# intellerce/controlanimate

Measured on AMD Instinct MI355X. Metric: frames_per_sec, higher is better.
Workload: dtype fp16

## Files before the change

### controlanimate_amd/_build.py

```python
from __future__ import annotations

import os
import subprocess
import sys
from concurrent.futures import ThreadPoolExecutor

CSRC = os.path.join(os.path.dirname(os.path.abspath(__file__)), "csrc")
LIB = os.path.join(CSRC, "libcontrolanimate_hip.so")
SOURCES = ["ca_gemm.hip", "ca_gemm_pp.hip", "ca_gemm_ar.hip", "ca_norm.hip", "ca_attention.hip", "ca_elementwise.hip", "ca_upscale.hip", "ca_color.hip", "ca_canny.hip", "ca_perceiver.hip", "ca_hed.hip", "ca_lineart.hip", "ca_mlsd.hip", "ca_softedge.hip", "ca_lineart_anime.hip", "ca_gfpgan.hip", "ca_depth.hip", "ca_openpose.hip", "ca_openpose_face.hip", "ca_openpose_hand.hip", "ca_normalbae.hip", "ca_retinaface.hip"]
HEADERS = ["ca_common.h", "ca_annot.h", "ca_gemm_core.h", "ca_gemm_plan.h", "ca_gemm_pp2.h", "ca_gemm_wres.h", "ca_gemm_ps.h", "ca_gemm_pq.h", "ca_gemm_ar.h", "ca_ff_fused.h", "ca_attn_out.h", "ca_tattn_fused.h", "ca_xattn_fused.h", "ca_gemm_seq.h", "ca_conv_wino.h", os.path.join("..", "..", "include", "controlanimate_hip.h")]
FLAGS = ["--offload-arch=gfx950", "-O3", "-std=c++17", "-fPIC", "-Wall", "-Wno-unused-function",
         "-mllvm", "-amdgpu-mfma-vgpr-form"]


EXTRA = {"ca_attention.hip": ["-fno-honor-nans"],
         "ca_color.hip": ["-ffp-contract=off"],
         "ca_hed.hip": ["-ffp-contract=off"],
         "ca_mlsd.hip": ["-ffp-contract=off"],
         "ca_softedge.hip": ["-ffp-contract=off"],
         "ca_gfpgan.hip": ["-ffp-contract=off"],
         "ca_depth.hip": ["-ffp-contract=off"],
         "ca_openpose.hip": ["-ffp-contract=off"]}
EXTRA["ca_openpose_face.hip"] = ["-ffp-contract=off"]
EXTRA["ca_openpose_hand.hip"] = ["-ffp-contract=off"]
EXTRA["ca_normalbae.hip"] = ["-ffp-contract=off"]
# ... 62 lines not shown
```

### controlanimate_amd/_capi.py

```python
from __future__ import annotations

import ctypes as C
import os

_HERE = os.path.dirname(os.path.abspath(__file__))
LIB_PATH = os.environ.get("CA_HIP_LIB") or os.path.join(_HERE, "csrc", "libcontrolanimate_hip.so")

CA_BF16, CA_F16 = 0, 1
CA_F32 = 2
CA_ACT_NONE, CA_ACT_SILU = 0, 1
CA_ACT_RELU = 4
CA_ACT_RELU6 = 5
CA_ACT_LEAKY02 = 6
CA_ACT_LEAKY001 = 7
CA_MLSD_TOPK = 200
CA_POSE_MAX_PEAKS, CA_POSE_MAX_PEOPLE, CA_POSE_AREA_TAPS = 64, 64, 8
CA_POSE_OVERFLOW_PEAKS, CA_POSE_OVERFLOW_PEOPLE = 1, 2
CA_POSE_OVERFLOW_FACES, CA_POSE_OVERFLOW_FACE_RESIZE = 4, 8
CA_FACE_SIZE, CA_FACE_HEAT, CA_FACE_PARTS, CA_FACE_MIN_SIDE, CA_FACE_SLOT_INTS = 384, 48, 71, 11, 8
CA_FACE_MODE_NONE, CA_FACE_MODE_LANCZOS4, CA_FACE_MODE_AREA = 0, 1, 2
CA_POSE_OVERFLOW_HANDS, CA_POSE_OVERFLOW_HAND_RESIZE = 16, 32
CA_HAND_PARTS, CA_HAND_HEAT_COLS, CA_HAND_MAP, CA_HAND_SCALES, CA_HAND_SLOT_INTS = 21, 24, 128, 4, 8
CA_HAND_MODE_NONE, CA_HAND_MODE_RESIZE, CA_HAND_MIN_BOX, CA_HAND_AREA_TAPS = 0, 1, 20, 16
CA_RFACE_MAX_CAND, CA_RFACE_HEAD_COLS, CA_RFACE_DET_COLS, CA_RFACE_MAX_FACES = 1024, 32, 15, 64
# ... 14 lines not shown
        ("a", C.c_void_p), ("a2", C.c_void_p), ("w", C.c_void_p), ("c", C.c_void_p),
        ("bias", C.c_void_p), ("rowbias", C.c_void_p), ("residual", C.c_void_p),
        ("lda", C.c_int64), ("lda2", C.c_int64), ("ldc", C.c_int64), ("ld_res", C.c_int64),
        ("ld_rowbias", C.c_int64),
        ("m", C.c_int32), ("n", C.c_int32), ("k1", C.c_int32), ("k2", C.c_int32),
        ("rows_per_group", C.c_int32),
        ("alpha", C.c_float), ("post_scale", C.c_float),
        ("act", C.c_int32), ("geglu", C.c_int32), ("out_f32", C.c_int32), ("dtype", C.c_int32),
        ("ln_stats", C.c_void_p), ("ln_colsum", C.c_void_p), ("ln_eps", C.c_float),
        ("workspace", C.c_void_p), ("workspace_bytes", C.c_int64),
        ("row_sums_out", C.c_void_p), ("ln_parts", C.c_int32),
        ("w_frag", C.c_void_p),
    ]


class FfArgs(C.Structure):
    _fields_ = [
        ("x", C.c_void_p), ("w1_frag", C.c_void_p), ("bias1", C.c_void_p), ("colsum1", C.c_void_p), ("ln_stats", C.c_void_p),
        ("w2_frag", C.c_void_p), ("bias2", C.c_void_p), ("residual", C.c_void_p), ("y", C.c_void_p),
        ("lda", C.c_int64), ("ldc", C.c_int64), ("ld_res", C.c_int64),
        ("m", C.c_int32), ("c", C.c_int32), ("inner", C.c_int32), ("ln_eps", C.c_float), ("dtype", C.c_int32),
        ("w_out_frag", C.c_void_p), ("bias_out", C.c_void_p), ("residual_out", C.c_void_p), ("ld_res_out", C.c_int64),
    ]


class TattnArgs(C.Structure):
    _fields_ = [
        ("x", C.c_void_p), ("w_frag", C.c_void_p), ("gamma", C.c_void_p), ("bias_pe", C.c_void_p), ("o", C.c_void_p),
        ("lda", C.c_int64), ("ldo", C.c_int64), ("ld_bias_pe", C.c_int64),
        ("batch", C.c_int32), ("frames", C.c_int32), ("tokens", C.c_int32), ("heads", C.c_int32), ("c", C.c_int32),
# ... 109 lines not shown


class Conv7x7Args(C.Structure):
    _fields_ = [
        ("x", C.c_void_p * 2), ("w", C.c_void_p * 2), ("bias", C.c_void_p * 2), ("y", C.c_void_p * 2),
        ("ldx", C.c_int64), ("ldy", C.c_int64),
        ("groups", C.c_int32), ("images", C.c_int32), ("h", C.c_int32), ("w_px", C.c_int32), ("cin", C.c_int32), ("cout", C.c_int32),
        ("relu", C.c_int32), ("dtype", C.c_int32),
    ]


SYMBOLS = {
    "ca_abi_version": (C.c_int, []),
    "ca_last_error": (C.c_char_p, []),
    "ca_gemm": (C.c_int, [C.POINTER(GemmArgs), C.c_void_p]),
    "ca_pack_w_frag": (C.c_int, [C.c_void_p, C.c_int32, C.c_int32, C.c_int32, C.c_void_p, C.c_void_p]),
    "ca_pack_w2_frag": (C.c_int, [C.c_void_p, C.c_int32, C.c_int32, C.c_void_p, C.c_void_p]),
    "ca_ff_fused": (C.c_int, [C.POINTER(FfArgs), C.c_void_p]),
    "ca_ff_fused_supported": (C.c_int, [C.POINTER(FfArgs)]),
    "ca_tattn_fused": (C.c_int, [C.POINTER(TattnArgs), C.c_void_p]),
    "ca_tattn_fused_supported": (C.c_int, [C.POINTER(TattnArgs)]),
    "ca_pack_w_tattn": (C.c_int, [C.c_void_p, C.c_int32, C.c_int32, C.c_void_p, C.c_void_p]),
    "ca_pack_w_out": (C.c_int, [C.c_void_p, C.c_int32, C.c_int32, C.c_void_p, C.c_void_p]),
    "ca_xattn_fused": (C.c_int, [C.POINTER(XattnArgs), C.c_void_p]),
    "ca_xattn_fused_supported": (C.c_int, [C.POINTER(XattnArgs)]),
    "ca_xattn_pack_w": (C.c_int, [C.c_void_p, C.c_int32, C.c_int32, C.c_void_p, C.c_void_p]),
    "ca_xattn_pack_kv": (C.c_int, [C.c_void_p, C.c_int64, C.c_int32, C.c_int32, C.c_int32, C.c_int32, C.c_float, C.c_int32, C.c_void_p, C.c_void_p]),
    "ca_gemm_ln_inline_supported": (C.c_int, [C.POINTER(GemmArgs)]),
    "ca_gemm_wants_finished_stats": (C.c_int, [C.POINTER(GemmArgs)]),
    "ca_ln_finish_sums": (C.c_int, [C.c_void_p, C.c_int, C.c_int64, C.c_int, C.c_float, C.c_void_p, C.c_void_p]),
# ... 174 lines not shown
```

### controlanimate_amd/context.py

```python
from __future__ import annotations

from dataclasses import dataclass, field
from typing import Optional

import torch


@dataclass
class ExecCtx:
    b: int
    f: int
    dtype: torch.dtype
    temb: torch.Tensor
    emb_groups: int
    ehs: Optional[torch.Tensor] = None
    frames_per_kv: int = 1
    kv_mod: int = 0
    gn_frames_per_stat: int = 1
    cache: dict = field(default_factory=dict)

    @property
    def images(self) -> int:
        return self.b * self.f

# ... 4 lines not shown
class Dispatch:
    gemm_ar = True
    ff_fused = True
    tattn_fused = True
    xattn_fused = True
    attn_out_fused = True
    xattn_ip_fused = True
    conv_winograd = True
    gn_winograd = True
    conv_up2_phase = True
    ln_row_sums = True
    repeat_kernel = True
    ln_fold = True
    cfg_shared = True
    cn_cfg_dedup = True
    pdc_block_fused = True
    dpt_head_fused = False
    pose_conv7_direct = True
    nbae_refine_fused = True
    controlnet_streams = 2


dispatch = Dispatch()
```

### controlanimate_amd/controlnet.py

```python
from __future__ import annotations

import dataclasses
from collections import OrderedDict

from typing import List, Optional, Sequence, Tuple, Union

import torch
from torch import nn

from . import kernels as K
from .context import ExecCtx
from .layers import HipConv1x1, HipConv3x3
from .unet import FrozenConfig, HipModelMixin, TimestepEmbedding, Timesteps
from .unet_blocks import UNetMidBlock3DCrossAttn, get_down_block


class ControlNetConditioningEmbedding(nn.Module):
    def __init__(self, conditioning_embedding_channels: int, conditioning_channels: int = 3,
                 block_out_channels: Tuple[int, ...] = (16, 32, 96, 256)):
        super().__init__()
        self.conv_in = HipConv3x3(conditioning_channels, block_out_channels[0])
        blocks = []
        for i in range(len(block_out_channels) - 1):
            blocks.append(HipConv3x3(block_out_channels[i], block_out_channels[i]))
# ... 173 lines not shown
            half = images // 2
            xh = self.conv_in.run(x[:half], residual=hint[:half])
            outs = [K.repeat_batch(xh)]
            x, o = first(xh, ctx, half_ctx=dataclasses.replace(ctx, b=half))
            outs += o
        else:
            x = self.conv_in.run(x, residual=hint)
            outs = [x]
        for blk in (self.down_blocks[1:] if shared else self.down_blocks):
            x, o = blk(x, ctx)
            outs += o
        x = self.mid_block(x, ctx)
        return outs, x, self.residual_scales(conditioning_scale, guess_mode), False

    @torch.no_grad()
    def apply_zero_convs(self, outs, x, scales, accumulate: Optional[Tuple[List[torch.Tensor], torch.Tensor]] = None, twice: bool = False):
        def one(zc, o, scale, prev):
            B_, h, w, c = o.shape
            rows = B_ * h * w
            a = o.view(rows, c)
            if not twice:
                return zc.run(a, alpha=scale, residual=None if prev is None else prev.view(rows, c)).view(B_, h, w, c)
            full = torch.empty((2 * B_, h, w, c), device=o.device, dtype=o.dtype)
            for hf in range(2):
                zc.run(a, alpha=scale, residual=None if prev is None else prev.view(2 * rows, c)[hf * rows:(hf + 1) * rows],
                       out=full.view(2 * rows, c)[hf * rows:(hf + 1) * rows])
            return full
        down = [one(zc, o, scales[i], None if accumulate is None else accumulate[0][i])
                for i, (zc, o) in enumerate(zip(self.controlnet_down_blocks, outs))]
        mid = one(self.controlnet_mid_block, x, scales[-1], None if accumulate is None else accumulate[1])
        return down, mid

    @torch.no_grad()
    def forward_nhwc(self, x: torch.Tensor, timestep, encoder_hidden_states: torch.Tensor, controlnet_cond: torch.Tensor,
                     conditioning_scale: float = 1.0, guess_mode: bool = False,
                     accumulate: Optional[Tuple[List[torch.Tensor], torch.Tensor]] = None, cfg_identical_halves: bool = False):
        outs, xm, scales, twice = self.forward_body(x, timestep, encoder_hidden_states, controlnet_cond, conditioning_scale, guess_mode,
                                                    cfg_identical_halves)
        return self.apply_zero_convs(outs, xm, scales, accumulate, twice)

    def forward(self, sample: torch.Tensor, timestep, encoder_hidden_states: torch.Tensor, controlnet_cond: torch.Tensor,
                conditioning_scale: float = 1.0, class_labels=None, timestep_cond=None, attention_mask=None,
                cross_attention_kwargs=None, guess_mode: bool = False, return_dict: bool = False):
        if not sample.is_cuda:
            raise RuntimeError("ControlNetModel runs on the HIP device only (no CPU fallback)")
# ... 22 lines not shown
        for n in self.nets:
            n.prepare(device, dtype)
        return self

    def forward_bodies(self, x, timestep, encoder_hidden_states, controlnet_cond: Sequence[torch.Tensor],
                       conditioning_scale: Sequence[float], guess_mode: bool = False, cfg_identical_halves: bool = False, streams=None):
        bodies = []
        for i, (net, cond, scale) in enumerate(zip(self.nets, controlnet_cond, conditioning_scale)):
            if streams:
                with torch.cuda.stream(streams[i % len(streams)]):
                    bodies.append(net.forward_body(x, timestep, encoder_hidden_states, cond, scale, guess_mode, cfg_identical_halves))
            else:
                bodies.append(net.forward_body(x, timestep, encoder_hidden_states, cond, scale, guess_mode, cfg_identical_halves))
        return bodies

    def finish(self, bodies, base: Optional[Tuple[List[torch.Tensor], torch.Tensor]] = None):
        acc = base
        for net, (outs, xm, scales, twice) in zip(self.nets, bodies):
            acc = net.apply_zero_convs(outs, xm, scales, acc, twice)
        return acc

    def forward_nhwc(self, x, timestep, encoder_hidden_states, controlnet_cond: Sequence[torch.Tensor],
                     conditioning_scale: Sequence[float], guess_mode: bool = False, cfg_identical_halves: bool = False):
        acc = None
        for net, cond, scale in zip(self.nets, controlnet_cond, conditioning_scale):
            acc = net.forward_nhwc(x, timestep, encoder_hidden_states, cond, scale, guess_mode, accumulate=acc,
                                   cfg_identical_halves=cfg_identical_halves)
        return acc

    def forward(self, sample, timestep, encoder_hidden_states, controlnet_cond, conditioning_scale, class_labels=None,
                timestep_cond=None, attention_mask=None, cross_attention_kwargs=None, guess_mode=False, return_dict=False):
        net0 = self.nets[0]
        net0._ensure_ready(sample.device)
        x = K.ncfhw_to_nhwc(sample.unsqueeze(2), net0.conv_in.cin_pad, net0.act_dtype)
# ... 3 lines not shown
```

### controlanimate_amd/controlresiduals_pipeline.py

```python
from __future__ import annotations

from typing import Callable, Dict, List, Optional, Sequence, Tuple

import numpy as np
import torch

from . import kernels as K
from .context import dispatch
from .controlnet import ControlNetModel, MultiControlNetModel


def _image_to_chw01(img) -> torch.Tensor:
    if torch.is_tensor(img):
        t = img.float()
        if t.dim() == 4:
            t = t[0]
        return t
    arr = np.asarray(img)
    if arr.ndim == 2:
        arr = np.stack([arr] * 3, axis=-1)
    t = torch.from_numpy(arr[..., :3].copy()).permute(2, 0, 1).float()
    return t / 255.0 if arr.dtype == np.uint8 else t


# ... 115 lines not shown
                                                    cfg_identical_halves=cfg_identical_halves, streams=streams if n_par > 1 else None)
            for s_ in streams[1:]:
                side.wait_stream(s_)
            if not capturing and n_par > 1:
                for i, (outs_, xm_, _, _) in enumerate(bodies):
                    if i % n_par:
                        for t_ in (*outs_, xm_):
                            t_.record_stream(side)
            if not fuse:
                down, mid = self.controlnet.finish(bodies)
                done = side.record_event()
        if not capturing:
            for s_ in streams:
                x_nhwc.record_stream(s_)

        def join(skips=None, mid_x=None):
            cur = torch.cuda.current_stream(dev)
            if not fuse:
                cur.wait_event(done)
                if not capturing:
                    for r in (*down, mid):
                        r.record_stream(cur)
                return down, mid
            if skips is None or mid_x is None:
                raise RuntimeError("a fused ControlNet join needs the UNet's skip tensors and mid-block output")
            side.wait_stream(cur)
            with torch.cuda.stream(side):
                d2, m2 = self.controlnet.finish(bodies, (list(skips), mid_x))
                fin = side.record_event()
            if not capturing:
                for s_ in (*skips, mid_x):
                    s_.record_stream(side)
            cur.wait_event(fin)
            if not capturing:
                for r in (*d2, m2):
                    r.record_stream(cur)
            return d2, m2

        join.fuse = fuse
        return join

    @torch.no_grad()
    def __call__(self, control_model_input: torch.Tensor, t, controlnet_prompt_embeds: torch.Tensor, frame_count: int,
                 image_embeds=None, do_classifier_free_guidance=True, guess_mode=True):
        b, c, f, h, w = control_model_input.shape
        if f != frame_count:
            raise ValueError("frame_count must equal the number of latent frames (SURVEY App. C-11)")
        net0 = self.controlnets[0]
        net0._ensure_ready(control_model_input.device)
        x = K.ncfhw_to_nhwc(control_model_input, net0.conv_in.cin_pad, net0.act_dtype)
        same = bool(self.detect_identical_halves and do_classifier_free_guidance and not guess_mode and b == 2
                    and torch.equal(control_model_input[0], control_model_input[1]))
        down, mid = self.residuals_nhwc(x, t, controlnet_prompt_embeds, guess_mode, cfg_identical_halves=same)

# ... 6 lines not shown
```

### controlanimate_amd/csrc/ca_gemm.hip

```cpp

#include "ca_gemm_plan.h"

namespace {
using namespace ca_gemm_detail;
#include "ca_conv_wino.h"

template <int DT, int BM, int BN, int WAVES_M, int WAVES_N, int MODE>
__global__ __launch_bounds__(256) void k_gemm(GemmKParams p) {
  constexpr int TM = BM / WAVES_M / 16;
  constexpr int TN = BN / WAVES_N / 16;
  constexpr int AI = BM / 32;
  constexpr int BI = BN / 32;
  static_assert(2 * (BM + BN) * BK >= BM * (BN + 8), "epilogue staging must fit");
  __shared__ __attribute__((aligned(16))) u16 smem[2 * (BM + BN) * BK];

  const int tid = threadIdx.x;
  const int lane = tid & 63;
  const int wid = tid >> 6;
  const int wm = wid / WAVES_N, wn = wid % WAVES_N;
  const int g = lane >> 4, l15 = lane & 15;

  const int tiles_n = (p.n + BN - 1) / BN;
  const unsigned bid = xcd_remap(blockIdx.x, gridDim.x);
  int tile_m, tile_n;
// ... 102 lines not shown
#pragma unroll
      for (int j = 0; j < TN; ++j) fb[j] = ld16(sb + lds_off(wn * TN * 16 + j * 16 + l15, s * 4 + g));
#pragma unroll
      for (int i = 0; i < TM; ++i)
#pragma unroll
        for (int j = 0; j < TN; ++j) acc[i][j] = Elem<DT>::mfma(fb[j], fa[i], acc[i][j]);
    }
    if (t + 1 < nt) store_tile(buf ^ 1);
    __syncthreads();
  }

  gemm_epilogue<DT, BM, BN, TM, TN>(p, acc, smem, m0, n0, wm, wn, l15, g, tid);
}


template <int DT, int BM, int BN, int WAVES_M, int WAVES_N, int MODE, int NBUF>
__global__ __launch_bounds__(256, NBUF == 1 ? (BN > 128 ? 3 : 4) : 2)
void k_gemm_dma(GemmKParams p) {
  static_assert(WAVES_M * WAVES_N == 4 && (NBUF == 1 || NBUF == 3), "instantiations: see above");
  constexpr int KT = BK;
  constexpr int CPR = KT / 8;
  constexpr int RPI = 64 / CPR;
  constexpr int NW = WAVES_M * WAVES_N, NT = NW * 64;
  constexpr int TM = BM / WAVES_M / 16;
  constexpr int TN = BN / WAVES_N / 16;
  constexpr int AG = BM / RPI / NW;
  constexpr int BG = BN / RPI / NW;
  constexpr int SMEM_ELEMS = NBUF * (BM + BN) * KT > BM * (BN + 8) ? NBUF * (BM + BN) * KT : BM * (BN + 8);
  auto swz = [](int row) { return (row >> 1) & 7; };
  auto lds_at = [&](int row, int chunk) { return row * KT + ((chunk ^ swz(row)) << 3); };
  __shared__ __attribute__((aligned(16))) u16 smem[SMEM_ELEMS];

  const int tid = threadIdx.x;
  const int lane = tid & 63;
  const int wid = tid >> 6;
  const int wm = wid / WAVES_N, wn = wid % WAVES_N;
  const int g = lane >> 4, l15 = lane & 15;

  const int tiles_n = (p.n + BN - 1) / BN;
  const int tiles_m = (p.m + BM - 1) / BM;
  unsigned bid = xcd_remap(blockIdx.x, gridDim.x);
  int split = 0;
  if (p.splits > 1) {
    split = bid / (unsigned)(tiles_m * tiles_n);
    bid -= split * (unsigned)(tiles_m * tiles_n);
  }
  int tile_m, tile_n;
  tile_coords(bid, tiles_m, tiles_n, tile_m, tile_n);
  const int m0 = tile_m * BM, n0 = tile_n * BN;

  const __amdgpu_buffer_rsrc_t rs_a = __builtin_amdgcn_make_buffer_rsrc((void*)p.a, 0, p.a_bytes, 0x00020000);
  const __amdgpu_buffer_rsrc_t rs_a2 = __builtin_amdgcn_make_buffer_rsrc((void*)(p.a2 ? p.a2 : p.a), 0, p.a2 ? p.a2_bytes : p.a_bytes, 0x00020000);
  const __amdgpu_buffer_rsrc_t rs_w = __builtin_amdgcn_make_buffer_rsrc((void*)p.w, 0, p.w_bytes, 0x00020000);

  const int r8 = lane / CPR, cp = lane % CPR;
  const int kc = p.c1 + p.c2;
// ... 130 lines not shown
  if (p.splits > 1) {
    float* slab = p.partial + (int64_t)split * p.m * p.n;
#pragma unroll
    for (int i = 0; i < TM; ++i) {
      const int m = m0 + wm * TM * 16 + i * 16 + l15;
      if (m >= p.m) continue;
#pragma unroll
      for (int j = 0; j < TN; ++j) {
        const int n = n0 + wn * TN * 16 + j * 16 + g * 4;
        if (n < p.n) *reinterpret_cast<f32x4*>(slab + (int64_t)m * p.n + n) = acc[i][j];
      }
    }
    return;
  }
  gemm_epilogue<DT, BM, BN, TM, TN, NT>(p, acc, smem, m0, n0, wm, wn, l15, g, tid);
}

template <int DT>
__global__ __launch_bounds__(256) void k_splitk_reduce(GemmKParams p) {
  const int64_t id = (int64_t)blockIdx.x * 256 + threadIdx.x;
  const int c8n = p.n >> 3;
  const int64_t m = id / c8n;
  if (m >= p.m) return;
  const int n = (int)(id - m * c8n) * 8;
  float v[8];
#pragma unroll
  for (int k = 0; k < 8; ++k) v[k] = 0.f;
  for (int sp = 0; sp < p.splits; ++sp) {
    const float* src = p.partial + ((int64_t)sp * p.m + m) * p.n + n;
    const f32x4 a = *reinterpret_cast<const f32x4*>(src), b = *reinterpret_cast<const f32x4*>(src + 4);
#pragma unroll
// ... 75 lines not shown
      return CA_OK;
  }
  CA_FAIL(CA_ERR_LAUNCH, "ca_gemm: no kernel for plan kind %d, tile %dx%d, %d stages", (int)g.kind, g.bm, g.bn, g.nbuf);
}

}

extern "C" int ca_gemm(const ca_gemm_args* a, void* stream) {
  DenseLaunch d;
  int rc = gemm_prepare(a, d);
  if (rc) return rc;
  hipStream_t st = (hipStream_t)stream;
  rc = a->dtype == CA_BF16 ? launch_gemm<CA_BF16, 0>(d.p, d.plan, st) : launch_gemm<CA_F16, 0>(d.p, d.plan, st);
  if (rc) return rc;
  CA_CHECK_LAUNCH("ca_gemm");
  return CA_OK;
}

extern "C" int64_t ca_gemm_workspace_bytes(const ca_gemm_args* a) {
  DenseLaunch d;
  return gemm_resolve(a, d) == CA_OK ? d.workspace : 0;
}

extern "C" int ca_gemm_row_sums_parts(const ca_gemm_args* a) {
  DenseLaunch d;
  DenseAsk ask{};
  ask.without_row_sums = true;
  return gemm_resolve(a, d, ask) == CA_OK ? row_sums_parts_of(d.p) : 0;
}

// ... 139 lines not shown
```

### controlanimate_amd/csrc/ca_gemm_core.h

```cpp
#pragma once
#include "ca_common.h"
#include <stdlib.h>

namespace ca_gemm_detail {


struct GemmKParams {
  const u16* a;
  const u16* a2;
  const u16* w;
  void* c;
  const float* bias;
  const float* rowbias;
  const float* ln_stats;
  const float* ln_colsum;
  const u16* res;
  int64_t lda, lda2, ldc, ld_res, ld_rowbias;
  unsigned a_bytes, a2_bytes, w_bytes;
  int m, n;
  int c1, c2;
  int taps;
  int kc_tiles;
  int hin, win, hout, wout, stride, ups, pad_lo;
  int rows_per_group;
// ... 2 lines not shown
  int splits;
  float* partial;
  int dbg;
  int tap_inner;
  float* row_sums;
  int ln_parts;
  int ln_inline;
  float ln_eps;
  const u16* wf;
  int w_group_rows;
  unsigned w_group_stride;
  int up2_rows, up2_tiles;
  unsigned up2_mag_w, up2_mag_h;
};

constexpr int BK = 64;

constexpr int GROUP_M = 8;
__device__ __forceinline__ void tile_coords(unsigned bid, int tiles_m, int tiles_n, int& tile_m, int& tile_n) {
  const unsigned gsz = GROUP_M * tiles_n;
  const unsigned group = bid / gsz, in = bid - group * gsz;
  const int first_m = group * GROUP_M;
  const int gm = tiles_m - first_m < GROUP_M ? tiles_m - first_m : GROUP_M;
  tile_m = first_m + in % gm;
  tile_n = in / gm;
}

__device__ __forceinline__ void k_tile_split(const GemmKParams& p, int t, int kct, int& tap, int& cc) {
  if (p.taps == 1) {
    tap = 0;
// ... 322 lines not shown
```

### controlanimate_amd/csrc/ca_gemm_plan.h

```cpp
#pragma once
#include "ca_gemm_core.h"

namespace ca_gemm_detail {

inline unsigned desc_bytes(int64_t elems) {
  const int64_t b = elems * 2;
  return (b > 0 && b < (int64_t)0xFFFFFF00ll) ? (unsigned)b : 0u;
}

inline bool dma_shape_ok(const GemmKParams& p) { return (p.c1 + p.c2) % BK == 0 && (p.c2 == 0 || p.c1 % BK == 0); }
inline bool dma_sizes_ok(const GemmKParams& p) { return p.a_bytes != 0 && p.w_bytes != 0 && (p.c2 == 0 || p.a2_bytes != 0); }
inline bool dma_capable(const GemmKParams& p) { return dma_shape_ok(p) && dma_sizes_ok(p); }

inline bool wres_eligible(const GemmKParams& p) {
  static const int wres_env = CA_KNOB("CA_GEMM_WRES", -1);
  const int kc = p.c1 + p.c2;
  return wres_env != 0 && kc == 320 && p.taps == 1 && (p.c2 == 0 || p.c1 % 32 == 0) && p.n % 160 == 0 && p.n / 160 <= 32 && !p.out_f32 &&
         p.splits <= 1 && !p.ln_parts && dma_sizes_ok(p) &&
         (!p.rowbias || p.rows_per_group % 32 == 0) &&
         act_out_fit31(p) &&
         (wres_env == 1 || p.m >= 16384);
}

inline bool ar_eligible(const GemmKParams& p, bool scratch) {
// ... 195 lines not shown
  if (p.ln_inline && p.wf) {
    if (ar_eligible(p, true)) d.workspace = (int64_t)p.m * 8;
    if (a->workspace && a->workspace_bytes >= (int64_t)p.m * 8) p.partial = reinterpret_cast<float*>(a->workspace);
  }
  d.plan = plan_gemm(p, 0);
  return CA_OK;
}

inline int gemm_prepare(const ca_gemm_args* a, DenseLaunch& d) {
  int rc = gemm_resolve(a, d);
  if (rc) return rc;
  CA_REQUIRE(!d.p.row_sums || row_sums_capable(d.p), "ca_gemm: row_sums_out is not available for this launch: ask ca_gemm_row_sums_parts() first");
  CA_REQUIRE(!d.p.ln_inline || wres_eligible(d.p), "ca_gemm: in-kernel LayerNorm statistics (ln_stats NULL) are not available for this launch: "
             "ask ca_gemm_ln_inline_supported() first and pass ln_stats otherwise");
  return CA_OK;
}

struct ConvGeom { int hl, wl, hout, wout; int64_t m; };
inline ConvGeom conv_geom(const ca_conv_args* a) {
  ConvGeom g;
  g.hl = a->hin << a->upsample, g.wl = a->win << a->upsample;
  const int pad = a->pad_asym ? 1 : 2;
  g.hout = (g.hl + pad - 3) / a->stride + 1;
  g.wout = (g.wl + pad - 3) / a->stride + 1;
  g.m = (int64_t)a->images * g.hout * g.wout;
  return g;
}
inline int64_t wino_tiles(const ca_conv_args* a, const ConvGeom& g) { return (int64_t)a->images * (g.hl / 2) * (g.wl / 2); }

inline int64_t wino_workspace_bytes(const ca_conv_args* a) {
// ... 118 lines not shown
```

### controlanimate_amd/kernels.py

```python
from __future__ import annotations

import ctypes as C
from typing import Optional

import torch

from . import _capi
from .context import dispatch
from ._capi import (AttnArgs, ConvArgs, ConvNarrowArgs, FfArgs, PerceiverAttnArgs, TattnArgs, XattnArgs, GemmArgs, GroupNormArgs, LayerNormArgs, CA_ACT_NONE,
                    CA_ACT_SILU, CA_BF16, CA_F16, check, lib)

ACT_NONE, ACT_SILU = CA_ACT_NONE, CA_ACT_SILU
ACT_QUICK_GELU, ACT_GELU = 2, 3
ACT_RELU = _capi.CA_ACT_RELU
ACT_RELU6 = _capi.CA_ACT_RELU6


def dt_code(dtype: torch.dtype) -> int:
    if dtype == torch.bfloat16:
        return CA_BF16
    if dtype == torch.float16:
        return CA_F16
    raise TypeError(f"activations must be bf16 or fp16, got {dtype}")

# ... 85 lines not shown
    if row_sums and dispatch.ln_row_sums and not geglu and not out_f32:
        parts = int(lib().ca_gemm_row_sums_parts(C.byref(args)))
        if parts > 0:
            rs = torch.empty((m, parts, 2), device=a.device, dtype=torch.float32)
            args.row_sums_out = _p(rs)
            out._row_sums = (rs, parts)
    wbytes = 0 if args.row_sums_out else int(lib().ca_gemm_workspace_bytes(C.byref(args)))
    if wbytes > 0:
        ws = torch.empty((wbytes,), device=a.device, dtype=torch.uint8)
        args.workspace, args.workspace_bytes = _p(ws), wbytes
    _record_plan(lib().ca_gemm_plan_name, args)
    check(lib().ca_gemm(C.byref(args), _stream()), "ca_gemm")
    return out


def attach_w_frag(w: torch.Tensor, geglu: bool = False) -> torch.Tensor:
    _req_cuda(w)
    if w.dim() != 2 or w.shape[1] != 320 or w.shape[0] % 320 != 0 or not w.is_contiguous() or w.dtype not in (torch.float16, torch.bfloat16):
        return w
    dst = torch.empty_like(w)
    check(lib().ca_pack_w_frag(w.data_ptr(), w.shape[0], w.shape[1], int(bool(geglu)), dst.data_ptr(), _stream()), "ca_pack_w_frag")
    w._frag = (dst, bool(geglu))
    return w


def ff_fused(x: torch.Tensor, w1_frag: torch.Tensor, bias1: torch.Tensor, colsum1: torch.Tensor, w2_frag: torch.Tensor,
             bias2: Optional[torch.Tensor], ln_eps: float, residual: Optional[torch.Tensor] = None,
             ln_stats: Optional[torch.Tensor] = None, *, w_out_frag: Optional[torch.Tensor] = None, bias_out: Optional[torch.Tensor] = None,
             residual_out: Optional[torch.Tensor] = None) -> Optional[torch.Tensor]:
    if not dispatch.ff_fused:
# ... 1845 lines not shown
```

### controlanimate_amd/unet.py

```python
from __future__ import annotations

from collections import OrderedDict

import dataclasses
import json
import os
from dataclasses import dataclass
from typing import Any, Dict, Optional, Tuple, Union

import torch
from torch import nn

from . import kernels as K
from .context import ExecCtx, dispatch
from .layers import HipGroupNorm, HipLinear, WeightArena, pack_concat_bias, pack_concat_rows
from .resnet import InflatedConv3d, InflatedGroupNorm, ResnetBlock3D
from .unet_blocks import UNetMidBlock3DCrossAttn, get_down_block, get_up_block


@dataclass
class UNet3DConditionOutput:
    sample: torch.Tensor


# ... 349 lines not shown
        shared = (cfg_identical_halves and dispatch.cfg_shared and b == 2 and getattr(first, "has_cross_attention", False) and
                  (not torch.is_tensor(timestep) or timestep.numel() == 1) and (timestep_cond is None or timestep_cond.shape[0] == 1))
        if shared:
            half_ctx = dataclasses.replace(ctx, b=1, temb=temb[:1], emb_groups=1)
            xh = self.conv_in.run(x[: x.shape[0] // 2])
            skips = [K.repeat_batch(xh)]
            x, outs = first(xh, ctx, half_ctx=half_ctx)
            skips += outs
        else:
            x = self.conv_in.run(x)
            skips = [x]
        for blk in (self.down_blocks[1:] if shared else self.down_blocks):
            x, outs = blk(x, ctx)
            skips += outs
        if callable(down_residuals) and getattr(down_residuals, "fuse", False):
            x = self.mid_block(x, ctx)
            skips, x = down_residuals(skips, x)
            for blk in self.up_blocks:
                n = len(blk.resnets)
                x = blk(x, skips[-n:], ctx)
                skips = skips[:-n]
            x = self.conv_norm_out.run(x, frames_per_stat=ctx.gn_frames_per_stat, act=K.ACT_SILU)
            return self.conv_out.run(x, out_f32=True)
        if callable(down_residuals):
            down_residuals, mid_residual = down_residuals()
        if down_residuals is not None:
            if len(down_residuals) != len(skips):
                raise ValueError("expected %d ControlNet residuals" % len(skips))
            skips = [K.add_bcast(s, r) for s, r in zip(skips, down_residuals)]
        x = self.mid_block(x, ctx)
# ... 72 lines not shown
```

### include/controlanimate_hip.h

```cpp
#ifndef CONTROLANIMATE_HIP_H
#define CONTROLANIMATE_HIP_H

#include <stdint.h>

#ifdef __cplusplus
extern "C" {
#endif

#define CA_ABI_VERSION 16

#define CA_BF16 0
#define CA_F16 1
#define CA_F32 2

#define CA_OK 0
#define CA_ERR_INVALID_ARG (-1)
#define CA_ERR_UNSUPPORTED (-2)
#define CA_ERR_LAUNCH (-3)

#define CA_ACT_NONE 0
#define CA_ACT_SILU 1
#define CA_ACT_QUICK_GELU 2
#define CA_ACT_GELU 3
#define CA_ACT_RELU 4
// ... 18 lines not shown
  float alpha, post_scale;
  int32_t act;
  int32_t geglu;
  int32_t out_f32;
  int32_t dtype;
  const float* ln_stats;
  const float* ln_colsum;
  float ln_eps;
  void* workspace;
  int64_t workspace_bytes;
  float* row_sums_out;
  int32_t ln_parts;
  const void* w_frag;
} ca_gemm_args;
int ca_gemm(const ca_gemm_args* args, void* stream);
int ca_pack_w_frag(const void* w, int32_t n, int32_t k, int32_t geglu, void* dst, void* stream);
typedef struct ca_ff_args {
  const void* x;
  const void* w1_frag;
  const float* bias1;
  const float* colsum1;
  const float* ln_stats;
  const void* w2_frag;
  const float* bias2;
  const void* residual;
  void* y;
  int64_t lda, ldc, ld_res;
  int32_t m, c, inner;
  float ln_eps;
  int32_t dtype;
// ... 542 lines not shown
```

Before: 15.91.

## Group ControlNet zero-conv GEMMs into one launch and start down-residuals early

```diff
diff --git a/controlanimate_amd/_build.py b/controlanimate_amd/_build.py
--- a/controlanimate_amd/_build.py
+++ b/controlanimate_amd/_build.py
@@ -8,7 +8,7 @@
 CSRC = os.path.join(os.path.dirname(os.path.abspath(__file__)), "csrc")
 LIB = os.path.join(CSRC, "libcontrolanimate_hip.so")
 SOURCES = ["ca_gemm.hip", "ca_gemm_pp.hip", "ca_gemm_ar.hip", "ca_norm.hip", "ca_attention.hip", "ca_elementwise.hip", "ca_upscale.hip", "ca_color.hip", "ca_canny.hip", "ca_perceiver.hip", "ca_hed.hip", "ca_lineart.hip", "ca_mlsd.hip", "ca_softedge.hip", "ca_lineart_anime.hip", "ca_gfpgan.hip", "ca_depth.hip", "ca_openpose.hip", "ca_openpose_face.hip", "ca_openpose_hand.hip", "ca_normalbae.hip", "ca_retinaface.hip"]
-HEADERS = ["ca_common.h", "ca_annot.h", "ca_gemm_core.h", "ca_gemm_plan.h", "ca_gemm_pp2.h", "ca_gemm_wres.h", "ca_gemm_ps.h", "ca_gemm_pq.h", "ca_gemm_ar.h", "ca_ff_fused.h", "ca_attn_out.h", "ca_tattn_fused.h", "ca_xattn_fused.h", "ca_gemm_seq.h", "ca_conv_wino.h", os.path.join("..", "..", "include", "controlanimate_hip.h")]
+HEADERS = ["ca_common.h", "ca_annot.h", "ca_gemm_core.h", "ca_gemm_plan.h", "ca_gemm_pp2.h", "ca_gemm_wres.h", "ca_gemm_ps.h", "ca_gemm_pq.h", "ca_gemm_ar.h", "ca_gemm_grouped.h", "ca_ff_fused.h", "ca_attn_out.h", "ca_tattn_fused.h", "ca_xattn_fused.h", "ca_gemm_seq.h", "ca_conv_wino.h", os.path.join("..", "..", "include", "controlanimate_hip.h")]
 FLAGS = ["--offload-arch=gfx950", "-O3", "-std=c++17", "-fPIC", "-Wall", "-Wno-unused-function",
          "-mllvm", "-amdgpu-mfma-vgpr-form"]
 
diff --git a/controlanimate_amd/_capi.py b/controlanimate_amd/_capi.py
--- a/controlanimate_amd/_capi.py
+++ b/controlanimate_amd/_capi.py
@@ -52,6 +52,15 @@
     ]
 
 
+class GemmGroupedProblem(C.Structure):
+    _fields_ = [
+        ("a", C.c_void_p), ("w", C.c_void_p), ("bias", C.c_void_p), ("c", C.c_void_p), ("residual", C.c_void_p),
+        ("c2", C.c_void_p), ("residual2", C.c_void_p),
+        ("lda", C.c_int64), ("ldc", C.c_int64), ("ld_res", C.c_int64), ("ldc2", C.c_int64), ("ld_res2", C.c_int64),
+        ("m", C.c_int32), ("n", C.c_int32), ("k", C.c_int32), ("alpha", C.c_float),
+    ]
+
+
 class FfArgs(C.Structure):
     _fields_ = [
         ("x", C.c_void_p), ("w1_frag", C.c_void_p), ("bias1", C.c_void_p), ("colsum1", C.c_void_p), ("ln_stats", C.c_void_p),
@@ -191,6 +200,9 @@
     "ca_abi_version": (C.c_int, []),
     "ca_last_error": (C.c_char_p, []),
     "ca_gemm": (C.c_int, [C.POINTER(GemmArgs), C.c_void_p]),
+    "ca_gemm_grouped": (C.c_int, [C.POINTER(GemmGroupedProblem), C.c_int32, C.c_int32, C.c_void_p]),
+    "ca_gemm_grouped_supported": (C.c_int, [C.POINTER(GemmGroupedProblem), C.c_int32, C.c_int32]),
+    "ca_gemm_grouped_plan_name": (C.c_int, [C.POINTER(GemmGroupedProblem), C.c_int32, C.c_int32, C.c_char_p, C.c_int32]),
     "ca_pack_w_frag": (C.c_int, [C.c_void_p, C.c_int32, C.c_int32, C.c_int32, C.c_void_p, C.c_void_p]),
     "ca_pack_w2_frag": (C.c_int, [C.c_void_p, C.c_int32, C.c_int32, C.c_void_p, C.c_void_p]),
     "ca_ff_fused": (C.c_int, [C.POINTER(FfArgs), C.c_void_p]),
diff --git a/controlanimate_amd/context.py b/controlanimate_amd/context.py
--- a/controlanimate_amd/context.py
+++ b/controlanimate_amd/context.py
@@ -42,6 +42,8 @@
     ln_fold = True
     cfg_shared = True
     cn_cfg_dedup = True
+    cn_zero_grouped = True
+    cn_zero_early = True
     pdc_block_fused = True
     dpt_head_fused = False
     pose_conv7_direct = True
diff --git a/controlanimate_amd/controlnet.py b/controlanimate_amd/controlnet.py
--- a/controlanimate_amd/controlnet.py
+++ b/controlanimate_amd/controlnet.py
@@ -211,21 +211,39 @@
         return outs, x, self.residual_scales(conditioning_scale, guess_mode), False
 
     @torch.no_grad()
-    def apply_zero_convs(self, outs, x, scales, accumulate: Optional[Tuple[List[torch.Tensor], torch.Tensor]] = None, twice: bool = False):
+    def apply_zero_convs(self, outs, x, scales, accumulate: Optional[Tuple[List[torch.Tensor], torch.Tensor]] = None, twice: bool = False,
+                         part: str = "all"):
+        from .context import dispatch
+        group = [] if dispatch.cn_zero_grouped else None
+
         def one(zc, o, scale, prev):
             B_, h, w, c = o.shape
             rows = B_ * h * w
             a = o.view(rows, c)
             if not twice:
-                return zc.run(a, alpha=scale, residual=None if prev is None else prev.view(rows, c)).view(B_, h, w, c)
+                res = None if prev is None else prev.view(rows, c)
+                if group is None:
+                    return zc.run(a, alpha=scale, residual=res).view(B_, h, w, c)
+                out = torch.empty((B_, h, w, c), device=o.device, dtype=o.dtype)
+                group.append(K.GroupedGemm(a, zc.w.t, zc.b.t, out.view(rows, c), res, alpha=scale))
+                return out
             full = torch.empty((2 * B_, h, w, c), device=o.device, dtype=o.dtype)
-            for hf in range(2):
-                zc.run(a, alpha=scale, residual=None if prev is None else prev.view(2 * rows, c)[hf * rows:(hf + 1) * rows],
-                       out=full.view(2 * rows, c)[hf * rows:(hf + 1) * rows])
+            halves = [(None if prev is None else prev.view(2 * rows, c)[hf * rows:(hf + 1) * rows], full.view(2 * rows, c)[hf * rows:(hf + 1) * rows])
+                      for hf in range(2)]
+            if group is None:
+                for res, out in halves:
+                    zc.run(a, alpha=scale, residual=res, out=out)
+            else:
+                group.append(K.GroupedGemm(a, zc.w.t, zc.b.t, halves[0][1], halves[0][0], halves[1][1], halves[1][0], alpha=scale))
             return full
-        down = [one(zc, o, scales[i], None if accumulate is None else accumulate[0][i])
-                for i, (zc, o) in enumerate(zip(self.controlnet_down_blocks, outs))]
-        mid = one(self.controlnet_mid_block, x, scales[-1], None if accumulate is None else accumulate[1])
+        down = mid = None
+        if part in ("all", "down"):
+            down = [one(zc, o, scales[i], None if accumulate is None else accumulate[0][i])
+                    for i, (zc, o) in enumerate(zip(self.controlnet_down_blocks, outs))]
+        if part in ("all", "mid"):
+            mid = one(self.controlnet_mid_block, x, scales[-1], None if accumulate is None else accumulate[1])
+        if group:
+            K.gemm_grouped(group)
         return down, mid
 
     @torch.no_grad()
@@ -278,10 +296,10 @@
                 bodies.append(net.forward_body(x, timestep, encoder_hidden_states, cond, scale, guess_mode, cfg_identical_halves))
         return bodies
 
-    def finish(self, bodies, base: Optional[Tuple[List[torch.Tensor], torch.Tensor]] = None):
+    def finish(self, bodies, base: Optional[Tuple[List[torch.Tensor], torch.Tensor]] = None, part: str = "all"):
         acc = base
         for net, (outs, xm, scales, twice) in zip(self.nets, bodies):
-            acc = net.apply_zero_convs(outs, xm, scales, acc, twice)
+            acc = net.apply_zero_convs(outs, xm, scales, acc, twice, part)
         return acc
 
     def forward_nhwc(self, x, timestep, encoder_hidden_states, controlnet_cond: Sequence[torch.Tensor],
diff --git a/controlanimate_amd/controlresiduals_pipeline.py b/controlanimate_amd/controlresiduals_pipeline.py
--- a/controlanimate_amd/controlresiduals_pipeline.py
+++ b/controlanimate_amd/controlresiduals_pipeline.py
@@ -153,6 +153,17 @@
             for s_ in streams:
                 x_nhwc.record_stream(s_)
 
+        early = {}
+
+        def start_down(skips):
+            cur = torch.cuda.current_stream(dev)
+            side.wait_stream(cur)
+            with torch.cuda.stream(side):
+                early["down"], _ = self.controlnet.finish(bodies, (list(skips), None), part="down")
+            if not capturing:
+                for s_ in skips:
+                    s_.record_stream(side)
+
         def join(skips=None, mid_x=None):
             cur = torch.cuda.current_stream(dev)
             if not fuse:
@@ -165,7 +176,11 @@
                 raise RuntimeError("a fused ControlNet join needs the UNet's skip tensors and mid-block output")
             side.wait_stream(cur)
             with torch.cuda.stream(side):
-                d2, m2 = self.controlnet.finish(bodies, (list(skips), mid_x))
+                if "down" in early:
+                    d2 = early.pop("down")
+                    _, m2 = self.controlnet.finish(bodies, (None, mid_x), part="mid")
+                else:
+                    d2, m2 = self.controlnet.finish(bodies, (list(skips), mid_x))
                 fin = side.record_event()
             if not capturing:
                 for s_ in (*skips, mid_x):
@@ -177,6 +192,7 @@
             return d2, m2
 
         join.fuse = fuse
+        join.start_down = start_down if fuse and dispatch.cn_zero_early else None
         return join
 
     @torch.no_grad()
diff --git a/controlanimate_amd/csrc/ca_gemm.hip b/controlanimate_amd/csrc/ca_gemm.hip
--- a/controlanimate_amd/csrc/ca_gemm.hip
+++ b/controlanimate_amd/csrc/ca_gemm.hip
@@ -140,9 +140,9 @@
 }
 
 
-template <int DT, int BM, int BN, int WAVES_M, int WAVES_N, int MODE, int NBUF>
-__global__ __launch_bounds__(256, NBUF == 1 ? (BN > 128 ? 3 : 4) : 2)
-void k_gemm_dma(GemmKParams p) {
+template <int DT, int BM, int BN, int WAVES_M, int WAVES_N, int MODE, int NBUF, bool SECOND = false>
+__device__ __forceinline__ void gemm_dma_tile(const GemmKParams& p, unsigned bid_raw, unsigned nblocks, void* c2 = nullptr, const u16* res2 = nullptr,
+                                              int64_t ldc2 = 0, int64_t ld_res2 = 0) {
   static_assert(WAVES_M * WAVES_N == 4 && (NBUF == 1 || NBUF == 3), "instantiations: see above");
   constexpr int KT = BK;
   constexpr int CPR = KT / 8;
@@ -165,7 +165,7 @@
 
   const int tiles_n = (p.n + BN - 1) / BN;
   const int tiles_m = (p.m + BM - 1) / BM;
-  unsigned bid = xcd_remap(blockIdx.x, gridDim.x);
+  unsigned bid = xcd_remap(bid_raw, nblocks);
   int split = 0;
   if (p.splits > 1) {
     split = bid / (unsigned)(tiles_m * tiles_n);
@@ -326,7 +326,21 @@
     return;
   }
   gemm_epilogue<DT, BM, BN, TM, TN, NT>(p, acc, smem, m0, n0, wm, wn, l15, g, tid);
-}
+  if (SECOND && c2) {
+    GemmKParams q = p;
+    q.c = c2, q.res = res2, q.ldc = ldc2, q.ld_res = ld_res2;
+    __syncthreads();
+    gemm_epilogue<DT, BM, BN, TM, TN, NT>(q, acc, smem, m0, n0, wm, wn, l15, g, tid);
+  }
+}
+
+template <int DT, int BM, int BN, int WAVES_M, int WAVES_N, int MODE, int NBUF>
+__global__ __launch_bounds__(256, NBUF == 1 ? (BN > 128 ? 3 : 4) : 2)
+void k_gemm_dma(GemmKParams p) {
+  gemm_dma_tile<DT, BM, BN, WAVES_M, WAVES_N, MODE, NBUF>(p, blockIdx.x, gridDim.x);
+}
+
+#include "ca_gemm_grouped.h"
 
 template <int DT>
 __global__ __launch_bounds__(256) void k_splitk_reduce(GemmKParams p) {
@@ -432,6 +446,30 @@
   rc = a->dtype == CA_BF16 ? launch_gemm<CA_BF16, 0>(d.p, d.plan, st) : launch_gemm<CA_F16, 0>(d.p, d.plan, st);
   if (rc) return rc;
   CA_CHECK_LAUNCH("ca_gemm");
+  return CA_OK;
+}
+
+extern "C" int ca_gemm_grouped_supported(const ca_gemm_grouped_problem* probs, int32_t count, int32_t dtype) {
+  GroupedTable t;
+  return grouped_capable(probs, count, dtype, t) ? 1 : 0;
+}
+
+extern "C" int ca_gemm_grouped(const ca_gemm_grouped_problem* probs, int32_t count, int32_t dtype, void* stream) {
+  GroupedTable t;
+  CA_REQUIRE(grouped_capable(probs, count, dtype, t), "ca_gemm_grouped: %d problems of dtype %d the grouped launch does not take (1..%d problems, fp16 / bf16, N and K "
+             "multiples of 64, leading dimensions multiples of 8, 16-byte aligned operands below 2 GB): ask ca_gemm_grouped_supported() first and run ca_gemm per "
+             "problem otherwise", count, dtype, GROUPED_MAX);
+  int rc = launch_gemm_grouped(t, dtype, (hipStream_t)stream);
+  if (rc) return rc;
+  CA_CHECK_LAUNCH("ca_gemm_grouped");
+  return CA_OK;
+}
+
+extern "C" int ca_gemm_grouped_plan_name(const ca_gemm_grouped_problem* probs, int32_t count, int32_t dtype, char* buf, int32_t len) {
+  CA_REQUIRE(buf && len > 0, "ca_gemm_grouped_plan_name: buffer");
+  GroupedTable t;
+  CA_REQUIRE(grouped_capable(probs, count, dtype, t), "ca_gemm_grouped_plan_name: problems the grouped launch does not take");
+  snprintf(buf, (size_t)len, "grouped128x64_r3");
   return CA_OK;
 }
 
diff --git a/controlanimate_amd/csrc/ca_gemm_core.h b/controlanimate_amd/csrc/ca_gemm_core.h
--- a/controlanimate_amd/csrc/ca_gemm_core.h
+++ b/controlanimate_amd/csrc/ca_gemm_core.h
@@ -40,6 +40,39 @@
   unsigned up2_mag_w, up2_mag_h;
 };
 
+constexpr int GROUPED_MAX = 32;
+struct GroupedProblem {
+  const u16* a;
+  const u16* w;
+  const float* bias;
+  u16* c;
+  const u16* res;
+  u16* c2;
+  const u16* res2;
+  int m, n, k;
+  int lda, ldc, ld_res, ldc2, ld_res2;
+  float alpha;
+};
+struct GroupedTable {
+  GroupedProblem prob[GROUPED_MAX];
+  unsigned first[GROUPED_MAX + 1];
+  int count;
+};
+static_assert(sizeof(GroupedTable) <= 3584, "the grouped table is a kernel argument: well under 4 KB");
+__host__ __device__ inline void grouped_fill(const GroupedProblem& g, GemmKParams& p) {
+  p = GemmKParams{};
+  p.a = g.a, p.w = g.w, p.c = g.c, p.bias = g.bias, p.res = g.res;
+  p.lda = g.lda, p.ldc = g.ldc, p.ld_res = g.ld_res;
+  p.a_bytes = (unsigned)(((int64_t)(g.m - 1) * g.lda + g.k) * 2);
+  p.w_bytes = (unsigned)((int64_t)g.n * g.k * 2);
+  p.m = g.m, p.n = g.n, p.c1 = g.k;
+  p.taps = 1;
+  p.kc_tiles = g.k / 64;
+  p.rows_per_group = 1;
+  p.alpha = g.alpha, p.post = 1.f;
+  p.splits = 1;
+}
+
 constexpr int BK = 64;
 
 constexpr int GROUP_M = 8;
diff --git a/controlanimate_amd/csrc/ca_gemm_grouped.h b/controlanimate_amd/csrc/ca_gemm_grouped.h
--- /dev/null
+++ b/controlanimate_amd/csrc/ca_gemm_grouped.h
@@ -0,0 +1,21 @@
+
+template <int DT>
+__global__ __launch_bounds__(256, 2) void k_gemm_grouped(GroupedTable t) {
+  const unsigned b = blockIdx.x;
+  int g = 0;
+#pragma unroll
+  for (int step = GROUPED_MAX / 2; step > 0; step >>= 1)
+    if (t.first[g + step] <= b) g += step;
+  g = __builtin_amdgcn_readfirstlane(g);
+  const GroupedProblem& q = t.prob[g];
+  GemmKParams p;
+  grouped_fill(q, p);
+  gemm_dma_tile<DT, 128, 64, 4, 1, 0, 3, true>(p, b - t.first[g], t.first[g + 1] - t.first[g], q.c2, q.res2, q.ldc2, q.ld_res2);
+}
+
+static int launch_gemm_grouped(const GroupedTable& t, int dtype, hipStream_t st) {
+  const dim3 grid(t.first[t.count]);
+  if (dtype == CA_BF16) hipLaunchKernelGGL((k_gemm_grouped<CA_BF16>), grid, dim3(256), 0, st, t);
+  else hipLaunchKernelGGL((k_gemm_grouped<CA_F16>), grid, dim3(256), 0, st, t);
+  return CA_OK;
+}
diff --git a/controlanimate_amd/csrc/ca_gemm_plan.h b/controlanimate_amd/csrc/ca_gemm_plan.h
--- a/controlanimate_amd/csrc/ca_gemm_plan.h
+++ b/controlanimate_amd/csrc/ca_gemm_plan.h
@@ -233,6 +233,52 @@
   CA_REQUIRE(!d.p.ln_inline || wres_eligible(d.p), "ca_gemm: in-kernel LayerNorm statistics (ln_stats NULL) are not available for this launch: "
              "ask ca_gemm_ln_inline_supported() first and pass ln_stats otherwise");
   return CA_OK;
+}
+
+inline bool grouped_problem_ok(const ca_gemm_grouped_problem& a, GroupedProblem& g) {
+  if (!a.a || !a.w || !a.c || a.m <= 0 || a.n <= 0 || a.k <= 0 || a.n % 64 != 0 || a.k % BK != 0) return false;
+  if (a.residual2 && !a.c2) return false;
+  const int64_t lds[5] = {a.lda, a.ldc, a.residual ? a.ld_res : 8, a.c2 ? a.ldc2 : 8, a.residual2 ? a.ld_res2 : 8};
+  for (int64_t ld : lds)
+    if (ld <= 0 || ld % 8 != 0 || ld >= (1ll << 31)) return false;
+  if (a.lda < a.k || a.ldc < a.n || (a.residual && a.ld_res < a.n) || (a.c2 && a.ldc2 < a.n) || (a.residual2 && a.ld_res2 < a.n)) return false;
+  if ((((uintptr_t)a.a | (uintptr_t)a.w | (uintptr_t)a.c | (uintptr_t)a.residual | (uintptr_t)a.c2 | (uintptr_t)a.residual2) & 15) != 0) return false;
+  if (((uintptr_t)a.bias & 15) != 0) return false;
+  g.a = (const u16*)a.a, g.w = (const u16*)a.w, g.bias = a.bias, g.c = (u16*)a.c, g.res = (const u16*)a.residual;
+  g.c2 = (u16*)a.c2, g.res2 = (const u16*)a.residual2;
+  g.m = a.m, g.n = a.n, g.k = a.k;
+  g.lda = (int)a.lda, g.ldc = (int)a.ldc, g.ld_res = a.residual ? (int)a.ld_res : 0;
+  g.ldc2 = a.c2 ? (int)a.ldc2 : 0, g.ld_res2 = a.residual2 ? (int)a.ld_res2 : 0;
+  g.alpha = a.alpha;
+  if (((int64_t)(a.m - 1) * a.lda + a.k) * 2 >= FIT31 || (int64_t)a.n * a.k * 2 >= FIT31) return false;
+  GemmKParams p;
+  grouped_fill(g, p);
+  if (!dma_capable(p) || !act_out_fit31(p) || p.w_bytes >= FIT31) return false;
+  if (g.c2) {
+    p.c = g.c2, p.res = g.res2, p.ldc = g.ldc2, p.ld_res = g.ld_res2;
+    if (!act_out_fit31(p)) return false;
+  }
+  return true;
+}
+inline bool grouped_capable(const ca_gemm_grouped_problem* probs, int count, int dtype, GroupedTable& t) {
+  if (!probs || count < 1 || count > GROUPED_MAX || (dtype != CA_F16 && dtype != CA_BF16)) return false;
+  int order[GROUPED_MAX];
+  for (int i = 0; i < count; ++i) {
+    int j = i;
+    for (; j > 0 && probs[order[j - 1]].m < probs[i].m; --j) order[j] = order[j - 1];
+    order[j] = i;
+  }
+  t = GroupedTable{};
+  t.count = count;
+  int64_t total = 0;
+  for (int i = 0; i < count; ++i) {
+    if (!grouped_problem_ok(probs[order[i]], t.prob[i])) return false;
+    t.first[i] = (unsigned)total;
+    total += (int64_t)ceil_div_i(t.prob[i].m, 128) * (t.prob[i].n / 64);
+    if (total >= (1ll << 31)) return false;
+  }
+  for (int i = count; i <= GROUPED_MAX; ++i) t.first[i] = (unsigned)total;
+  return true;
 }
 
 struct ConvGeom { int hl, wl, hout, wout; int64_t m; };
diff --git a/controlanimate_amd/kernels.py b/controlanimate_amd/kernels.py
--- a/controlanimate_amd/kernels.py
+++ b/controlanimate_amd/kernels.py
@@ -123,6 +123,47 @@
     return out
 
 
+class GroupedGemm:
+    __slots__ = ("a", "w", "bias", "out", "residual", "out2", "residual2", "alpha")
+
+    def __init__(self, a, w, bias, out, residual=None, out2=None, residual2=None, alpha: float = 1.0):
+        self.a, self.w, self.bias, self.out, self.residual, self.out2, self.residual2, self.alpha = a, w, bias, out, residual, out2, residual2, float(alpha)
+
+
+def gemm_grouped(problems) -> bool:
+    problems = list(problems)
+    if not problems:
+        return True
+    dt = problems[0].a.dtype
+    arr = (_capi.GemmGroupedProblem * len(problems))()
+    for g, q in zip(arr, problems):
+        _req_cuda(q.a, q.w, q.bias, q.out, q.residual, q.out2, q.residual2)
+        assert q.a.dim() == 2 and q.a.stride(1) == 1 and q.w.dim() == 2 and q.w.is_contiguous() and q.a.dtype == dt and q.w.dtype == dt
+        m, k = q.a.shape
+        n = q.w.shape[0]
+        assert q.w.shape[1] == k and (q.bias is None or (q.bias.dtype == torch.float32 and q.bias.numel() == n))
+        assert q.out2 is not None or q.residual2 is None
+        for t in (q.out, q.residual, q.out2, q.residual2):
+            assert t is None or (tuple(t.shape) == (m, n) and t.stride(1) == 1 and t.dtype == dt)
+        g.a, g.w, g.bias, g.c, g.residual, g.c2, g.residual2 = _p(q.a), _p(q.w), _p(q.bias), _p(q.out), _p(q.residual), _p(q.out2), _p(q.residual2)
+        g.lda, g.ldc = q.a.stride(0), q.out.stride(0)
+        g.ld_res = q.residual.stride(0) if q.residual is not None else 0
+        g.ldc2 = q.out2.stride(0) if q.out2 is not None else 0
+        g.ld_res2 = q.residual2.stride(0) if q.residual2 is not None else 0
+        g.m, g.n, g.k, g.alpha = m, n, k, q.alpha
+    if lib().ca_gemm_grouped_supported(arr, len(problems), dt_code(dt)):
+        if _plan_sink is not None:
+            buf = C.create_string_buffer(64)
+            _plan_sink.append(buf.value.decode() if lib().ca_gemm_grouped_plan_name(arr, len(problems), dt_code(dt), buf, 64) == 0 else "?")
+        check(lib().ca_gemm_grouped(arr, len(problems), dt_code(dt), _stream()), "ca_gemm_grouped")
+        return True
+    for q in problems:
+        gemm(q.a, q.w, bias=q.bias, residual=q.residual, alpha=q.alpha, out=q.out)
+        if q.out2 is not None:
+            gemm(q.a, q.w, bias=q.bias, residual=q.residual2, alpha=q.alpha, out=q.out2)
+    return False
+
+
 def attach_w_frag(w: torch.Tensor, geglu: bool = False) -> torch.Tensor:
     _req_cuda(w)
     if w.dim() != 2 or w.shape[1] != 320 or w.shape[0] % 320 != 0 or not w.is_contiguous() or w.dtype not in (torch.float16, torch.bfloat16):
diff --git a/controlanimate_amd/unet.py b/controlanimate_amd/unet.py
--- a/controlanimate_amd/unet.py
+++ b/controlanimate_amd/unet.py
@@ -387,6 +387,8 @@
             x, outs = blk(x, ctx)
             skips += outs
         if callable(down_residuals) and getattr(down_residuals, "fuse", False):
+            if getattr(down_residuals, "start_down", None) is not None:
+                down_residuals.start_down(skips)
             x = self.mid_block(x, ctx)
             skips, x = down_residuals(skips, x)
             for blk in self.up_blocks:
diff --git a/include/controlanimate_hip.h b/include/controlanimate_hip.h
--- a/include/controlanimate_hip.h
+++ b/include/controlanimate_hip.h
@@ -56,6 +56,21 @@
   const void* w_frag;
 } ca_gemm_args;
 int ca_gemm(const ca_gemm_args* args, void* stream);
+typedef struct ca_gemm_grouped_problem {
+  const void* a;
+  const void* w;
+  const float* bias;
+  void* c;
+  const void* residual;
+  void* c2;
+  const void* residual2;
+  int64_t lda, ldc, ld_res, ldc2, ld_res2;
+  int32_t m, n, k;
+  float alpha;
+} ca_gemm_grouped_problem;
+int ca_gemm_grouped(const ca_gemm_grouped_problem* problems, int32_t count, int32_t dtype, void* stream);
+int ca_gemm_grouped_supported(const ca_gemm_grouped_problem* problems, int32_t count, int32_t dtype);
+int ca_gemm_grouped_plan_name(const ca_gemm_grouped_problem* problems, int32_t count, int32_t dtype, char* buf, int32_t len);
 int ca_pack_w_frag(const void* w, int32_t n, int32_t k, int32_t geglu, void* dst, void* stream);
 typedef struct ca_ff_args {
   const void* x;
```

Result: no change. 16.04, median of 6 (+0.8%).
